# haoheliu/ssr_eval

Hardware: AMD Instinct MI355X
Metric: utterance-pairs/sec (LSD+SSIM, 48kHz, n_fft=2048) (higher is better)
Workload: dtype f64

## Files before the change

### ssr_eval_amd/csrc/ssr_stft_wave.h

```cpp
#pragma once
#include "ssr_stft.h"


constexpr int SSR_W_N = 2048, SSR_W_L = 64, SSR_W_P = 32;
constexpr int SSR_W_TWP = 7 * 32 + 12 * 64;
SSR_DEV int ssr_wpad(int i) { return i + (i >> 5); }
constexpr int SSR_W_PN = SSR_W_N + (SSR_W_N >> 5) + 1;

template <typename T> SSR_DEV cx<T> ssr_w32(int m) {
  constexpr double c[22] = {1.0, 0.98078528040323044913, 0.92387953251128675613, 0.83146961230254523708, 0.70710678118654752440,
                            0.55557023301960222474, 0.38268343236508977173, 0.19509032201612826785, 0.0,
                            -0.19509032201612826785, -0.38268343236508977173, -0.55557023301960222474, -0.70710678118654752440,
                            -0.83146961230254523708, -0.92387953251128675613, -0.98078528040323044913, -1.0,
                            -0.98078528040323044913, -0.92387953251128675613, -0.83146961230254523708, -0.70710678118654752440,
                            -0.55557023301960222474};
  constexpr double s[22] = {0.0, -0.19509032201612826785, -0.38268343236508977173, -0.55557023301960222474, -0.70710678118654752440,
                            -0.83146961230254523708, -0.92387953251128675613, -0.98078528040323044913, -1.0,
                            -0.98078528040323044913, -0.92387953251128675613, -0.83146961230254523708, -0.70710678118654752440,
                            -0.55557023301960222474, -0.38268343236508977173, -0.19509032201612826785, 0.0,
                            0.19509032201612826785, 0.38268343236508977173, 0.55557023301960222474, 0.70710678118654752440,
                            0.83146961230254523708};
  return {(T)c[m], (T)s[m]};
}

template <typename T, int NZ = 32> SSR_DEV void ssr_dft32(cx<T>* v) {
  const T h = (T)0.70710678118654752440;
  static_assert(NZ == 32 || (NZ > 8 && NZ <= 16), "full, or two non-zero row groups");
  SSR_UNROLL for (int n2 = 0; n2 < 8; ++n2) {
    cx<T> t[4] = {v[n2], v[8 + n2], v[16 + n2], v[24 + n2]};
    if (NZ == 32) {
      ssr_bfly4(t);
    } else if (8 + n2 < NZ) {
      const cx<T> r = cmul_negi(t[1]);
      t[2] = csub(t[0], t[1]); t[3] = csub(t[0], r);
      t[1] = cadd(t[0], r);    t[0] = cadd(t[0], v[8 + n2]);
    } else {
      t[1] = t[0]; t[2] = t[0]; t[3] = t[0];
    }
    SSR_UNROLL for (int k1 = 0; k1 < 4; ++k1) {
      const int m = n2 * k1;
      cx<T> x = t[k1];
      if (m == 0) {
      } else if (m == 8) {
        x = cmul_negi(x);
      } else if (m == 16) {
        x = {-x.x, -x.y};
      } else if (m == 4) {
        x = {h * (x.x + x.y), h * (x.y - x.x)};
      } else if (m == 12) {
        x = {h * (x.y - x.x), -h * (x.x + x.y)};
      } else if (m == 20) {
        x = {-h * (x.x + x.y), h * (x.x - x.y)};
      } else {
        x = cmul(x, ssr_w32<T>(m));
      }
      v[8 * k1 + n2] = x;
    }
  }
  SSR_UNROLL for (int k1 = 0; k1 < 4; ++k1) ssr_bfly8(v + 8 * k1);
}
SSR_DEV constexpr int ssr_dft32_freq(int rho) { return (rho >> 3) + 4 * (rho & 7); }

struct SsrTrue { static constexpr bool value = true; };
struct SsrFalse { static constexpr bool value = false; };

template <typename T, bool SUMS> struct SsrWaveRegs {
  cx<T> v[SSR_W_P];
  T tx[SSR_W_P];
  float pa[SSR_W_P], pb[SSR_W_P];
  T wl[SSR_W_P / 2];
  cx<T> tw1[7];
  cx<T> tw2[12];
  double lsd_total;
};

template <typename T, bool SPLIT> struct SsrWaveLds {
  static constexpr size_t bytes() { return sizeof(double) * 4 + sizeof(int) * 8 + sizeof(T) * (SPLIT ? 1 : 2) * SSR_W_PN; }
  double* sc1; int* nz; T* re; T* im;
  SSR_MEMBER explicit SsrWaveLds(char* base) {
    sc1 = reinterpret_cast<double*>(base);
    nz = reinterpret_cast<int*>(sc1 + 4);
    re = reinterpret_cast<T*>(nz + 8);
    im = SPLIT ? re : re + SSR_W_PN;
  }
  SSR_MEMBER bool nonzero(int which, int par) const {
    int f = nz[which * 2 + par];
#ifndef SSR_HOST_EMU
    f = __builtin_amdgcn_readfirstlane(f);
#endif
    return f != 0;
  }
};

template <typename T> struct SsrWaveBuf { T* re; T* im; };

template <typename T, bool SPLIT> constexpr size_t ssr_stft_wave_sums_offset() { return (SsrWaveLds<T, SPLIT>::bytes() + 7) & ~(size_t)7; }
template <typename T, bool SPLIT, bool SUMS> constexpr size_t ssr_stft_wave_lds_bytes() {
  return SUMS ? ssr_stft_wave_sums_offset<T, SPLIT>() + 6 * 64 * sizeof(double) : SsrWaveLds<T, SPLIT>::bytes();
}

struct SsrWaveBase { int st0, ld8, st1; };
SSR_DEV SsrWaveBase ssr_wave_bases(int tid) {
  return {33 * tid, tid + (tid >> 5), 264 * (tid >> 5) + (tid & 31)};
}
SSR_DEV constexpr int ssr_w_off_st0(int i) { return ssr_dft32_freq(i); }
SSR_DEV constexpr int ssr_w_off_ld8(int i) { return 66 * (i >> 3) + 264 * (i & 7); }
SSR_DEV constexpr int ssr_w_off_st1(int i) { return 528 * (i >> 3) + 33 * (i & 7); }

#define SSR_W_EXCHANGE_G(blk, regs, L, WB, WO, RBASES, RIDX, EXTRA)                                       \
  if constexpr (!SPLIT) {                                                                                 \
    SSR_WPHASE(blk, regs, { const int w_ = ssr_wave_bases(tid & 63).WB;                                        \
      SSR_UNROLL for (int i = 0; i < SSR_W_P; ++i) { (L).re[w_ + WO(i)] = R.v[i].x; (L).im[w_ + WO(i)] = R.v[i].y; } }); \
    SSR_WPHASE(blk, regs, { SSR_SCHED_BARRIER(); EXTRA; const auto r_ = RBASES(tid & 63);                    \
      SSR_UNROLL for (int i = 0; i < SSR_W_P; ++i) R.v[i] = {(L).re[RIDX(r_, i)], (L).im[RIDX(r_, i)]}; });   \
  } else {                                                                                                \
    SSR_WPHASE(blk, regs, { const int w_ = ssr_wave_bases(tid & 63).WB;                                        \
      SSR_UNROLL for (int i = 0; i < SSR_W_P; ++i) (L).re[w_ + WO(i)] = R.v[i].x; });                     \
    SSR_WPHASE(blk, regs, { SSR_SCHED_BARRIER(); EXTRA; const auto r_ = RBASES(tid & 63);                    \
      SSR_UNROLL for (int i = 0; i < SSR_W_P; ++i) R.tx[i] = (L).re[RIDX(r_, i)]; });                     \
    SSR_WPHASE(blk, regs, { const int w_ = ssr_wave_bases(tid & 63).WB;                                        \
      SSR_UNROLL for (int i = 0; i < SSR_W_P; ++i) (L).re[w_ + WO(i)] = R.v[i].y; });                     \
    SSR_WPHASE(blk, regs, { const auto r_ = RBASES(tid & 63);                                                \
      SSR_UNROLL for (int i = 0; i < SSR_W_P; ++i) R.v[i] = {R.tx[i], (L).re[RIDX(r_, i)]}; });           \
  }
#define SSR_W_RIDX_LD8(b_, i) ((b_).ld8 + ssr_w_off_ld8(i))
#define SSR_W_EXCHANGE(blk, regs, L, WB, WO, RB, RO, EXTRA) SSR_W_EXCHANGE_G(blk, regs, L, WB, WO, ssr_wave_bases, SSR_W_RIDX_##RB##_##RO, EXTRA)
#define SSR_W_RIDX_ld8_ssr_w_off_ld8(b_, i) SSR_W_RIDX_LD8(b_, i)

struct SsrWavePBase { int ld8, p2, p3; };
SSR_DEV int ssr_wave_pj3(int tid) { return tid == 0 ? 128 : 256 - tid; }
SSR_DEV SsrWavePBase ssr_wave_pbases(int tid) {
  return {tid + (tid >> 5), ssr_wpad(192 - tid), ssr_wpad(ssr_wave_pj3(tid))};
}
SSR_DEV int ssr_w_rd_paired(const SsrWavePBase& B, int i) {
  const int b = i >> 3, q = i & 7;
  return (b == 0 ? B.ld8 : b == 1 ? B.ld8 + 66 : b == 2 ? B.p2 : B.p3) + 264 * q;
}
#define SSR_W_RIDX_PAIRED(b_, i) ssr_w_rd_paired(b_, i)
#define SSR_W_LOAD_TW2_PAIRED { const int t_ = tid & 63; const unsigned l_ = SSR_UIDX(t_);                       \
    const unsigned o2_ = SSR_UIDX(t_ == 0 ? 192 : 64 - t_); const unsigned o3_ = SSR_UIDX(t_ == 0 ? -192 : 64 - t_); \
    SSR_UNROLL for (int i = 0; i < 6; ++i) R.tw2[i] = VT.at(l_ + (SSR_W_N + 224 + 64 * i));                       \
    SSR_UNROLL for (int i = 6; i < 9; ++i) R.tw2[i] = VT.at(o2_ + (SSR_W_N + 224 + 64 * i));                      \
    SSR_UNROLL for (int i = 9; i < 12; ++i) R.tw2[i] = VT.at(o3_ + (SSR_W_N + 224 + 64 * i)); }

#define SSR_W_LOAD_TW1 { const unsigned l_ = SSR_UIDX(tid & 31); \
                         SSR_UNROLL for (int q = 1; q < 8; ++q) R.tw1[q - 1] = VT.at(l_ + (SSR_W_N + 32 * (q - 1))); }
#define SSR_W_LOAD_TW2 { const unsigned l_ = SSR_UIDX(tid & 63); \
                         SSR_UNROLL for (int i = 0; i < 12; ++i) R.tw2[i] = VT.at(l_ + (SSR_W_N + 224 + 64 * i)); }
#define SSR_W_FFT_TAIL(blk, BLK0, regs, L, EXTRA2)                                                                        \
  SSR_W_FFT_TAIL_X(blk, BLK0, regs, L, SSR_W_EXCHANGE(blk, regs, L, st1, ssr_w_off_st1, ld8, ssr_w_off_ld8, SSR_W_LOAD_TW2 EXTRA2))
#define SSR_W_FFT_TAIL_PAIRED(blk, BLK0, regs, L)                                                                         \
  SSR_W_FFT_TAIL_X(blk, BLK0, regs, L, SSR_W_EXCHANGE_G(blk, regs, L, st1, ssr_w_off_st1, ssr_wave_pbases, SSR_W_RIDX_PAIRED, SSR_W_LOAD_TW2_PAIRED))
#define SSR_W_FFT_TAIL_X(blk, BLK0, regs, L, EXCH2)                                                                       \
  blk = BLK0; ssr_launder(blk);                                                                                     \
  SSR_W_EXCHANGE(blk, regs, L, st0, ssr_w_off_st0, ld8, ssr_w_off_ld8, SSR_W_LOAD_TW1);                             \
   \
  SSR_WPHASE(blk, regs, {                                                                                           \
    SSR_UNROLL for (int b = 0; b < 4; ++b) {                                                                        \
      SSR_UNROLL for (int q = 1; q < 8; ++q) R.v[8 * b + q] = cmul(R.v[8 * b + q], R.tw1[q - 1]);                   \
      ssr_bfly8(R.v + 8 * b);                                                                                       \
    }                                                                                                               \
  });                                                                                                               \
  blk = BLK0; ssr_launder(blk);                                                                                     \
  EXCH2;                                                                                                            \
    \
  SSR_WPHASE(blk, regs, {                                                                                           \
    SSR_UNROLL for (int b = 0; b < 4; ++b) {                                                                        \
      cx<T>* x = R.v + 8 * b;                                                                                       \
      const cx<T> w1 = R.tw2[3 * b], w2 = R.tw2[3 * b + 1], w4 = R.tw2[3 * b + 2];                                  \
      x[1] = cmul(x[1], w1);                                                                                        \
      x[2] = cmul(x[2], w2);                                                                                        \
      x[4] = cmul(x[4], w4);                                                                                        \
      const cx<T> w3 = cmul(w1, w2);                                                                                \
      x[3] = cmul(x[3], w3);                                                                                        \
      x[5] = cmul(x[5], cmul(w1, w4));                                                                              \
      x[6] = cmul(x[6], cmul(w2, w4));                                                                              \
      x[7] = cmul(x[7], cmul(w3, w4));                                                                              \
      ssr_bfly8(x);                                                                                                 \
    }                                                                                                               \
  });

template <typename T, int WHICH = 3, typename REGS>
SSR_DEV void ssr_wave_prefetch(const SsrStftParams<T>& p, REGS& R, int tid, const SsrView<float>& va, const SsrView<float>& vb,
                               int u, int n, int n_frames) {
  const int t_c = (u < n_frames) ? u : n_frames - 1;
  const int base = t_c * p.hop - SSR_W_N / 2;
  if (base >= 0 && base + SSR_W_N <= n) {
    SSR_UNROLL for (int r = 0; r < SSR_W_P; ++r) {
      if (WHICH & 1) R.pa[r] = va.at(SSR_UIDX(tid + 64 * r), base);
      if (WHICH & 2) R.pb[r] = vb.at(SSR_UIDX(tid + 64 * r), base);
    }
  } else {
    SSR_UNROLL for (int r = 0; r < SSR_W_P; ++r) {
      const unsigned m = SSR_UIDX(ssr_reflect(base + tid + 64 * r, n));
      if (WHICH & 1) R.pa[r] = va.at(m);
      if (WHICH & 2) R.pb[r] = vb.at(m);
    }
  }
}

template <typename REGS> SSR_DEV void ssr_wave_flags(REGS& R, int tid, int* nz, int par) {
  SSR_UNROLL for (int r = 0; r < SSR_W_P; ++r) { ssr_touch(R.pa[r]); ssr_touch(R.pb[r]); }
  unsigned ora = 0u, orb = 0u;
  SSR_UNROLL for (int r = 1; r < SSR_W_P; ++r) { ora |= ssr_mag_bits(R.pa[r]); orb |= ssr_mag_bits(R.pb[r]); }
  ora |= (tid == 0) ? 0u : ssr_mag_bits(R.pa[0]);
  orb |= (tid == 0) ? 0u : ssr_mag_bits(R.pb[0]);
  SSR_WAVE_ANY_STORE(tid, ora != 0u, nz + par);
  SSR_WAVE_ANY_STORE(tid, orb != 0u, nz + 2 + par);
}

template <typename T, bool SUMS, bool SPLIT, int MAG = -1, typename BLK>
SSR_BODY void ssr_stft_wave_body(const SsrStftParams<T>& p, BLK& blk, int chunk, int item, char* lds_base) {
  constexpr int N = SSR_W_N, F = N / 2 + 1;
  using Regs = SsrWaveRegs<T, SUMS>;
  SsrWaveLds<T, SPLIT> L(lds_base);
  const int n = p.len[item], hop = p.hop;
  const int n_frames = ssr_num_frames_dev(n, N, hop);
  const int S = p.interleave > 1 ? p.interleave : 1;
  const int span0 = (chunk / S) * S * p.units_per_chunk;
  const int u0 = span0 + chunk % S;
  const int u1 = (span0 + S * p.units_per_chunk < n_frames) ? span0 + S * p.units_per_chunk : n_frames;
  const float* sa = p.a + p.a_off[item];
  const float* sb = p.b + p.b_off[item];
  const int64_t row0 = p.frame_off[item];
  double* part = p.part ? p.part + ((int64_t)item * p.n_chunks + chunk) * SSR_NPART : nullptr;
  const int mask = SUMS ? p.metric_mask : (p.metric_mask & SSR_M_LSD);
  const bool want_lsd = mask & SSR_M_LSD;
  const SsrView<float> va(sa, n), vb(sb, n);
  const SsrView<T> vw(p.window, N);
  const SsrView<cx<T>> vt(p.tw, N + SSR_W_TWP);

  double* lsum = reinterpret_cast<double*>(lds_base + ssr_stft_wave_sums_offset<T, SPLIT>());
  SSR_REGS(Regs, regs, blk);
  SSR_WPHASE(blk, regs, {
    R.lsd_total = 0.0;
    if constexpr (SUMS) for (int q = 0; q < 6; ++q) lsum[64 * q + tid] = 0.0;
    if (tid == 0) L.sc1[0] = 0.0;
    if (u0 < u1) {
      ssr_wave_prefetch<T>(p, R, tid, va, vb, u0, n, n_frames);
      SSR_UNROLL for (int r = 0; r < SSR_W_P / 2; ++r) R.wl[r] = vw.at(SSR_UIDX(tid + 64 * r));
    }
    SSR_VMEM_DRAIN();
  });

  BLK blk0 = blk;
  for (int u = u0, it = 0; u < u1; u += S, ++it) {
    blk = blk0; ssr_launder(blk);
    SSR_WPHASE(blk, regs, {
      ssr_wave_flags(R, tid, L.nz, it & 1);
      SSR_UNROLL for (int r = 0; r < SSR_W_P; ++r) {
        const T w = (r < SSR_W_P / 2) ? R.wl[r] : (T)0.5 - R.wl[r - SSR_W_P / 2];
        R.v[r] = {(T)R.pa[r] * w, (T)R.pb[r] * w};
      }
      ssr_dft32(R.v);
      if (want_lsd && it > 0 && tid == 0) R.lsd_total += sqrt(L.sc1[0] / (double)F);
    });
#define VT vt
    SSR_W_FFT_TAIL_PAIRED(blk, blk0, regs, L);
#undef VT

    blk = blk0; ssr_launder(blk);
    const int64_t OP = p.out_pitch ? p.out_pitch : F;
    float* ra0 = p.out_a ? p.out_a + (row0 + u) * OP : nullptr;
    float* rb0 = p.out_b ? p.out_b + (row0 + u) * OP : nullptr;
    SSR_WPHASE(blk, regs, {
      SSR_SCHED_BARRIER();
      double acc[7] = {0.0, 0.0, 0.0, 0.0, 0.0, 0.0, 0.0};
      const int par = it & 1;
      const bool a_nz = L.nonzero(0, par), b_nz = L.nonzero(1, par);
      const bool both = a_nz && b_nz;
      const bool store = MAG < 0 ? p.out_kind == SSR_OUT_MAG : MAG != 0;
      const SsrRwView<float> wa(ra0, store ? F : 0), wb(rb0, (store && rb0 != nullptr) ? F : 0);
      const int lane4 = 4 * tid, lane4_2 = 4 * (192 - tid), lane4_3 = 4 * ssr_wave_pj3(tid);
      auto bin_off = [&](int b, int q) -> int {
        return (b == 0 ? lane4 : b == 1 ? lane4 + 256 : b == 2 ? lane4_2 : lane4_3) + 1024 * q;
      };
      cx<T> rot4 = {(T)0, (T)0};
      if (tid == 0) {
        rot4 = R.v[28];
        const cx<T> t29 = R.v[29], t30 = R.v[30], t31 = R.v[31];
        R.v[31] = R.v[0]; R.v[30] = R.v[7]; R.v[29] = R.v[6]; R.v[28] = R.v[5];
        R.v[7] = t31; R.v[6] = t30; R.v[5] = t29;
      }
      constexpr int G = 2;
      constexpr int PF1 = SUMS ? 1 : 0;
      auto bins = [&](auto fast_tag) {
        constexpr bool FAST = decltype(fast_tag)::value;
        SSR_UNROLL for (int b = 0; b < 4; ++b) SSR_UNROLL for (int q0 = 0; q0 < 4; q0 += G) {
          cx<T> zn[G];
          SSR_UNROLL for (int q = 0; q < G; ++q) zn[q] = R.v[8 * (3 - b) + 7 - (q0 + q)];
          SSR_UNROLL for (int q = 0; q < G; q += 2) {
            const cx<T> zk0 = R.v[8 * b + q0 + q], zk1 = R.v[8 * b + q0 + q + 1];
            f2 e, t;
            if constexpr (FAST) {
              ssr_pair_bins2_fast<T, SUMS>(acc, zk0, zn[q], zk1, zn[q + 1], e, t);
            } else {
              float e0, t0, e1, t1;
              ssr_pair_bin<T, 0, true>(mask, acc, zk0, zn[q], a_nz, b_nz, e0, t0);
              ssr_pair_bin<T, 0, true>(mask, acc, zk1, zn[q + 1], a_nz, b_nz, e1, t1);
              e = f2_make(e0, e1); t = f2_make(t0, t1);
            }
            if (store) {
              wa.st_raw(bin_off(b, q0 + q), e.x);
              wa.st_raw(bin_off(b, q0 + q + 1), e.y);
              wb.st_raw(bin_off(b, q0 + q), t.x);
              wb.st_raw(bin_off(b, q0 + q + 1), t.y);
            }
          }
          if (b == 0 && q0 + G == 4) {
            if (tid == 0) {
              const cx<T> zq = R.v[4];
              float e, t;
              ssr_pair_bin<T, 0, true>(mask, acc, zq, zq, a_nz, b_nz, e, t);
              if (store) { wa.st_raw(4 * (N / 2), e); wb.st_raw(4 * (N / 2), t); }
              R.v[4] = rot4;
            }
          }
          if (b == PF1 && q0 + G == 4) {
            SSR_SCHED_BARRIER();
            ssr_wave_prefetch<T, 1>(p, R, tid, va, vb, u + S, n, n_frames);
            SSR_SCHED_BARRIER();
          }
          if (b == PF1 + 1 && q0 + G == 4) {
            SSR_SCHED_BARRIER();
            ssr_wave_prefetch<T, 2>(p, R, tid, va, vb, u + S, n, n_frames);
            SSR_SCHED_BARRIER();
          }
          if (b == PF1 + 2 && q0 + G == 4) {
            SSR_SCHED_BARRIER();
            SSR_UNROLL for (int r = 0; r < SSR_W_P / 2; ++r) R.wl[r] = vw.at(SSR_UIDX(tid + 64 * r));
            SSR_SCHED_BARRIER();
          }
        }
      };
      constexpr int FULL = SUMS ? (SSR_M_LSD | SSR_M_LOG_SISPEC | SSR_M_SISPEC) : SSR_M_LSD;
      if (both && (mask & 7) == FULL) bins(SsrTrue{});
      else bins(SsrFalse{});
      if (want_lsd) SSR_WAVE_SUM_STORE(tid, 64, acc[0], L.sc1);
      if constexpr (SUMS)
        for (int q = 0; q < 6; ++q) SSR_LDS_ACCUM(lsum + 64 * q + tid, acc[1 + q]);
    });
  }

  if (part == nullptr) return;
  if constexpr (SUMS) {
    for (int q = 0; q < 6; ++q) {
      SSR_WPHASE(blk, regs, SSR_WAVE_SUM_STORE(tid, 64, lsum[64 * q + tid], L.sc1 + 1));
      SSR_WPHASE(blk, regs, if (tid == 0) part[1 + q] = L.sc1[1]);
    }
  } else {
    SSR_WPHASE(blk, regs, if (tid == 0) for (int q = 0; q < 6; ++q) part[1 + q] = 0.0);
  }
  SSR_WPHASE(blk, regs, if (tid == 0) {
    double lsd = R.lsd_total;
    if (want_lsd && u1 > u0) lsd += sqrt(L.sc1[0] / (double)F);
    part[0] = lsd;
    part[7] = 0.0;
  });
}
```

Measured before the change: 344,300.

## Stream next frame's samples into LDS via buffer_load_lds DMA instead of registers

For the float64 split-LDS path, the next frame's two input signals are fetched straight into the exchange LDS array with buffer_load_lds (16-byte when aligned and inside, 4-byte otherwise, reflected at edges). The per-thread pa/pb register arrays are removed from the register struct in that path, which frees VGPRs. The old mid-loop register prefetch is replaced by a single request issued after the FFT, with an explicit vmcnt wait before use. An optional resident mode keeps window and twiddle registers loaded across iterations. The cost is hand-computed waitcnt values and LDS reuse that must not overlap with exchange reads.

```diff
diff --git a/ssr_eval_amd/csrc/ssr_stft_wave.h b/ssr_eval_amd/csrc/ssr_stft_wave.h
--- a/ssr_eval_amd/csrc/ssr_stft_wave.h
+++ b/ssr_eval_amd/csrc/ssr_stft_wave.h
@@ -64,10 +64,12 @@
 struct SsrTrue { static constexpr bool value = true; };
 struct SsrFalse { static constexpr bool value = false; };
 
-template <typename T, bool SUMS> struct SsrWaveRegs {
+template <bool PRE> struct SsrWaveSamples { float pa[SSR_W_P], pb[SSR_W_P]; };
+template <> struct SsrWaveSamples<false> {};
+
+template <typename T, bool SUMS, bool PRE = true> struct SsrWaveRegs : SsrWaveSamples<PRE> {
   cx<T> v[SSR_W_P];
   T tx[SSR_W_P];
-  float pa[SSR_W_P], pb[SSR_W_P];
   T wl[SSR_W_P / 2];
   cx<T> tw1[7];
   cx<T> tw2[12];
@@ -148,12 +150,12 @@
 #define SSR_W_LOAD_TW2 { const unsigned l_ = SSR_UIDX(tid & 63); \
                          SSR_UNROLL for (int i = 0; i < 12; ++i) R.tw2[i] = VT.at(l_ + (SSR_W_N + 224 + 64 * i)); }
 #define SSR_W_FFT_TAIL(blk, BLK0, regs, L, EXTRA2)                                                                        \
-  SSR_W_FFT_TAIL_X(blk, BLK0, regs, L, SSR_W_EXCHANGE(blk, regs, L, st1, ssr_w_off_st1, ld8, ssr_w_off_ld8, SSR_W_LOAD_TW2 EXTRA2))
-#define SSR_W_FFT_TAIL_PAIRED(blk, BLK0, regs, L)                                                                         \
-  SSR_W_FFT_TAIL_X(blk, BLK0, regs, L, SSR_W_EXCHANGE_G(blk, regs, L, st1, ssr_w_off_st1, ssr_wave_pbases, SSR_W_RIDX_PAIRED, SSR_W_LOAD_TW2_PAIRED))
-#define SSR_W_FFT_TAIL_X(blk, BLK0, regs, L, EXCH2)                                                                       \
+  SSR_W_FFT_TAIL_X(blk, BLK0, regs, L, SSR_W_LOAD_TW1, SSR_W_EXCHANGE(blk, regs, L, st1, ssr_w_off_st1, ld8, ssr_w_off_ld8, SSR_W_LOAD_TW2 EXTRA2))
+#define SSR_W_FFT_TAIL_PAIRED(blk, BLK0, regs, L, EXTRA1)                                                                 \
+  SSR_W_FFT_TAIL_X(blk, BLK0, regs, L, EXTRA1, SSR_W_EXCHANGE_G(blk, regs, L, st1, ssr_w_off_st1, ssr_wave_pbases, SSR_W_RIDX_PAIRED, SSR_W_LOAD_TW2_PAIRED))
+#define SSR_W_FFT_TAIL_X(blk, BLK0, regs, L, EXTRA1, EXCH2)                                                               \
   blk = BLK0; ssr_launder(blk);                                                                                     \
-  SSR_W_EXCHANGE(blk, regs, L, st0, ssr_w_off_st0, ld8, ssr_w_off_ld8, SSR_W_LOAD_TW1);                             \
+  SSR_W_EXCHANGE(blk, regs, L, st0, ssr_w_off_st0, ld8, ssr_w_off_ld8, EXTRA1);                                     \
    \
   SSR_WPHASE(blk, regs, {                                                                                           \
     SSR_UNROLL for (int b = 0; b < 4; ++b) {                                                                        \
@@ -209,11 +211,91 @@
   SSR_WAVE_ANY_STORE(tid, orb != 0u, nz + 2 + par);
 }
 
+template <typename T, bool SPLIT> constexpr bool ssr_wave_dma() { return SPLIT && sizeof(T) == 8; }
+#ifndef SSR_WAVE_RESIDENT
+#define SSR_WAVE_RESIDENT 0
+#endif
+static_assert(2 * SSR_W_N * sizeof(float) <= SSR_W_PN * sizeof(double), "both signals of a frame fit the float64 exchange array");
+static_assert((sizeof(double) * 4 + sizeof(int) * 8) % 16 == 0, "the exchange array starts on a 16-byte boundary");
+
+#ifndef SSR_HOST_EMU
+typedef __attribute__((address_space(3))) float* SsrLdsF;
+SSR_DEV void ssr_lds_dma16(const SsrView<float>& v, SsrLdsF dst, int voff, int soff) {
+  __builtin_amdgcn_raw_ptr_buffer_load_lds(v.rsrc, dst, 16, voff, soff, 0, 0);
+}
+SSR_DEV void ssr_lds_dma4(const SsrView<float>& v, SsrLdsF dst, int voff, int soff) {
+  __builtin_amdgcn_raw_ptr_buffer_load_lds(v.rsrc, dst, 4, voff, soff, 0, 0);
+}
+#endif
+
+template <typename T>
+SSR_DEV void ssr_wave_request(const SsrStftParams<T>& p, float* ls, int tid, const float* sa, const float* sb, const SsrView<float>& va,
+                              const SsrView<float>& vb, int u, int n, int n_frames) {
+  const int t_c = (u < n_frames) ? u : n_frames - 1;
+  const int base = t_c * p.hop - SSR_W_N / 2;
+  const bool inside = base >= 0 && base + SSR_W_N <= n;
+#ifdef SSR_HOST_EMU
+  (void)sa; (void)sb;
+  for (int r = 0; r < SSR_W_P; ++r) {
+    const unsigned m = SSR_UIDX(inside ? base + tid + 64 * r : ssr_reflect(base + tid + 64 * r, n));
+    ls[tid + 64 * r] = va.at(m);
+    ls[SSR_W_N + tid + 64 * r] = vb.at(m);
+  }
+#else
+  const bool wide = inside && (((uintptr_t)(sa + base) | (uintptr_t)(sb + base)) & 15) == 0;
+  const SsrLdsF l3 = (SsrLdsF)ls;
+  if (wide) {
+    SSR_UNROLL for (int k = 0; k < 8; ++k) ssr_lds_dma16(va, l3 + 256 * k, 16 * tid, 4 * (base + 256 * k));
+    SSR_UNROLL for (int k = 0; k < 8; ++k) ssr_lds_dma16(vb, l3 + SSR_W_N + 256 * k, 16 * tid, 4 * (base + 256 * k));
+  } else if (inside) {
+    SSR_UNROLL for (int r = 0; r < SSR_W_P; ++r) {
+      ssr_lds_dma4(va, l3 + 64 * r, 4 * (tid + 64 * r), 4 * base);
+      ssr_lds_dma4(vb, l3 + SSR_W_N + 64 * r, 4 * (tid + 64 * r), 4 * base);
+    }
+  } else {
+    SSR_UNROLL for (int r = 0; r < SSR_W_P; ++r) {
+      const int m4 = 4 * ssr_reflect(base + tid + 64 * r, n);
+      ssr_lds_dma4(va, l3 + 64 * r, m4, 0);
+      ssr_lds_dma4(vb, l3 + SSR_W_N + 64 * r, m4, 0);
+    }
+  }
+#endif
+}
+
+#ifdef SSR_HOST_EMU
+SSR_DEV void ssr_wave_lds_drain() {}
+#else
+SSR_DEV void ssr_wave_lds_drain() {
+  SSR_SCHED_BARRIER();
+  __builtin_amdgcn_s_waitcnt(0xC07F);
+  SSR_SCHED_FENCE();
+  SSR_SCHED_BARRIER();
+}
+#endif
+template <int MAG, bool RES = false> constexpr int ssr_wave_dma_behind() { return (MAG != 0 ? 2 * 16 + 2 : 0) + (RES ? 0 : SSR_W_P / 2); }
+#ifdef SSR_HOST_EMU
+template <int MAG, bool RES> SSR_DEV void ssr_wave_dma_wait() {}
+#else
+template <int MAG, bool RES> SSR_DEV void ssr_wave_dma_wait() {
+  static_assert(MAG >= 0, "the count needs to know at compile time whether rows are stored");
+  constexpr int n = ssr_wave_dma_behind<MAG, RES>();
+  static_assert(n < 64, "vmcnt is six bits");
+  SSR_SCHED_BARRIER();
+  __builtin_amdgcn_s_waitcnt(0x0F70 | (n & 15) | ((n >> 4) << 14));
+  SSR_SCHED_FENCE();
+  SSR_SCHED_BARRIER();
+}
+#endif
+
 template <typename T, bool SUMS, bool SPLIT, int MAG = -1, typename BLK>
 SSR_BODY void ssr_stft_wave_body(const SsrStftParams<T>& p, BLK& blk, int chunk, int item, char* lds_base) {
   constexpr int N = SSR_W_N, F = N / 2 + 1;
-  using Regs = SsrWaveRegs<T, SUMS>;
+  constexpr bool DMA = ssr_wave_dma<T, SPLIT>();
+  constexpr bool RES = DMA && (SSR_WAVE_RESIDENT & 1);
+  constexpr bool RES1 = DMA && (SSR_WAVE_RESIDENT & 2);
+  using Regs = SsrWaveRegs<T, SUMS, !DMA>;
   SsrWaveLds<T, SPLIT> L(lds_base);
+  float* ls = reinterpret_cast<float*>(L.re);
   const int n = p.len[item], hop = p.hop;
   const int n_frames = ssr_num_frames_dev(n, N, hop);
   const int S = p.interleave > 1 ? p.interleave : 1;
@@ -232,31 +314,41 @@
 
   double* lsum = reinterpret_cast<double*>(lds_base + ssr_stft_wave_sums_offset<T, SPLIT>());
   SSR_REGS(Regs, regs, blk);
+#define VT vt
   SSR_WPHASE(blk, regs, {
     R.lsd_total = 0.0;
     if constexpr (SUMS) for (int q = 0; q < 6; ++q) lsum[64 * q + tid] = 0.0;
     if (tid == 0) L.sc1[0] = 0.0;
     if (u0 < u1) {
-      ssr_wave_prefetch<T>(p, R, tid, va, vb, u0, n, n_frames);
+      if constexpr (DMA) ssr_wave_request<T>(p, ls, tid, sa, sb, va, vb, u0, n, n_frames);
+      else ssr_wave_prefetch<T>(p, R, tid, va, vb, u0, n, n_frames);
       SSR_UNROLL for (int r = 0; r < SSR_W_P / 2; ++r) R.wl[r] = vw.at(SSR_UIDX(tid + 64 * r));
+      if constexpr (RES1) SSR_W_LOAD_TW1
     }
     SSR_VMEM_DRAIN();
   });
+#undef VT
 
   BLK blk0 = blk;
   for (int u = u0, it = 0; u < u1; u += S, ++it) {
     blk = blk0; ssr_launder(blk);
     SSR_WPHASE(blk, regs, {
-      ssr_wave_flags(R, tid, L.nz, it & 1);
+      SsrWaveSamples<true> smp;
+      if constexpr (DMA) {
+        ssr_wave_dma_wait<MAG, RES>();
+        SSR_UNROLL for (int r = 0; r < SSR_W_P; ++r) { smp.pa[r] = ls[tid + 64 * r]; smp.pb[r] = ls[SSR_W_N + tid + 64 * r]; }
+      }
+      auto& X = [&]() -> auto& { if constexpr (DMA) return smp; else return R; }();
+      ssr_wave_flags(X, tid, L.nz, it & 1);
       SSR_UNROLL for (int r = 0; r < SSR_W_P; ++r) {
         const T w = (r < SSR_W_P / 2) ? R.wl[r] : (T)0.5 - R.wl[r - SSR_W_P / 2];
-        R.v[r] = {(T)R.pa[r] * w, (T)R.pb[r] * w};
+        R.v[r] = {(T)X.pa[r] * w, (T)X.pb[r] * w};
       }
       ssr_dft32(R.v);
       if (want_lsd && it > 0 && tid == 0) R.lsd_total += sqrt(L.sc1[0] / (double)F);
     });
 #define VT vt
-    SSR_W_FFT_TAIL_PAIRED(blk, blk0, regs, L);
+    SSR_W_FFT_TAIL_PAIRED(blk, blk0, regs, L, if constexpr (!RES1) SSR_W_LOAD_TW1);
 #undef VT
 
     blk = blk0; ssr_launder(blk);
@@ -265,6 +357,12 @@
     float* rb0 = p.out_b ? p.out_b + (row0 + u) * OP : nullptr;
     SSR_WPHASE(blk, regs, {
       SSR_SCHED_BARRIER();
+      if constexpr (DMA) {
+        SSR_UNROLL for (int i = 0; i < SSR_W_P; ++i) { ssr_touch(R.v[i].x); ssr_touch(R.v[i].y); }
+        ssr_wave_lds_drain();
+        ssr_wave_request<T>(p, ls, tid, sa, sb, va, vb, u + S, n, n_frames);
+        SSR_SCHED_BARRIER();
+      }
       double acc[7] = {0.0, 0.0, 0.0, 0.0, 0.0, 0.0, 0.0};
       const int par = it & 1;
       const bool a_nz = L.nonzero(0, par), b_nz = L.nonzero(1, par);
@@ -316,22 +414,25 @@
               R.v[4] = rot4;
             }
           }
-          if (b == PF1 && q0 + G == 4) {
-            SSR_SCHED_BARRIER();
-            ssr_wave_prefetch<T, 1>(p, R, tid, va, vb, u + S, n, n_frames);
-            SSR_SCHED_BARRIER();
+          if constexpr (!DMA) {
+            if (b == PF1 && q0 + G == 4) {
+              SSR_SCHED_BARRIER();
+              ssr_wave_prefetch<T, 1>(p, R, tid, va, vb, u + S, n, n_frames);
+              SSR_SCHED_BARRIER();
+            }
+            if (b == PF1 + 1 && q0 + G == 4) {
+              SSR_SCHED_BARRIER();
+              ssr_wave_prefetch<T, 2>(p, R, tid, va, vb, u + S, n, n_frames);
+              SSR_SCHED_BARRIER();
+            }
           }
-          if (b == PF1 + 1 && q0 + G == 4) {
-            SSR_SCHED_BARRIER();
-            ssr_wave_prefetch<T, 2>(p, R, tid, va, vb, u + S, n, n_frames);
-            SSR_SCHED_BARRIER();
-          }
-          if (b == PF1 + 2 && q0 + G == 4) {
+          if (!RES && b == PF1 + 2 && q0 + G == 4) {
             SSR_SCHED_BARRIER();
             SSR_UNROLL for (int r = 0; r < SSR_W_P / 2; ++r) R.wl[r] = vw.at(SSR_UIDX(tid + 64 * r));
             SSR_SCHED_BARRIER();
           }
         }
+        if constexpr (DMA && !RES && !FAST) { SSR_UNROLL for (int r = 0; r < SSR_W_P / 2; ++r) ssr_touch(R.wl[r]); }
       };
       constexpr int FULL = SUMS ? (SSR_M_LSD | SSR_M_LOG_SISPEC | SSR_M_SISPEC) : SSR_M_LSD;
       if (both && (mask & 7) == FULL) bins(SsrTrue{});
@@ -342,6 +443,7 @@
     });
   }
 
+  if constexpr (DMA) { SSR_WPHASE(blk, regs, SSR_VMEM_DRAIN()); }
   if (part == nullptr) return;
   if constexpr (SUMS) {
     for (int q = 0; q < 6; ++q) {
```

After: 346,900, median of 6. About the same (+0.8%).
